# SamArgt/AudioSourceSep

Measured on AMD Instinct MI355X. Metric: Glow fwd+logdet passes/sec on 64×64×1 mel tiles (K=32,L=3), 1→8 MI355X, higher is better.
Workload: dtype f16x3

## Files before the change

audiosourcesep_amd/csrc/glowk_act_scale.h:

```cpp
#pragma once
#define GLOWK_ACT_SCALE 4.0f
```

audiosourcesep_amd/csrc/glowk_co.h:

```cpp
#pragma once
#include "glowk_kernels.h"

constexpr int CO_PX = 128;
constexpr int CO_PSTR = 132;

template <int KIN, int MOUT, int NF, int MODE>
struct RingC {
  static constexpr int MODE7 = net_dir<MODE>;
  using S = RingS<KIN, MOUT, NF, MODE7, 2>;
  static constexpr bool FUSE = (MODE & NET_FUSE) != 0;
  static constexpr bool SAVE = MODE7 == NET_FWD_SAVE, BWD = MODE7 == NET_BWD;
  static constexpr bool MERGE = S::NMT <= 3;
  static constexpr bool M0LAST = S::NMT % 3 == 2;
  static constexpr bool STORE = (MODE & NET_STORE) != 0;
  static constexpr int MODEX = net_dir<MODE> | (MODE & NET_STORE);
  static constexpr int NFH = S::NFH, NRB = S::NRB, NMT = S::NMT, KS = S::KS;
  static constexpr int UNITP = S::MAINP / 2;
  static constexpr int UNIT4 = S::MAIN4 / 2;
  static constexpr int PPW = UNITP / 4;
  static constexpr int NG = NFH / 2;
  static constexpr int K1PW = (S::K1P + 3) / 4;
  static constexpr int EPN = BWD ? 0 : S::EPN;
  static constexpr int MASKN = BWD ? 2 * 4 * NF * 64 : 0;
  static constexpr size_t LDS_BYTES = (size_t)3 * UNIT4 * 16 + (size_t)2 * S::K14 * 16 + (size_t)EPN * 4 + (size_t)MASKN * 2 +
// ... 258 lines not shown
  if constexpr (G::BWD) {
    stage4<NF / 2, 65>(reinterpret_cast<const float4*>(a.mask1 + (size_t)blockIdx.x * 4 * NF * 64), reinterpret_cast<float4*>(mkl), c.w4, c.voff);
    stage4<NF / 2, 66>(reinterpret_cast<const float4*>(a.mask2 + (size_t)blockIdx.x * 4 * NF * 64), reinterpret_cast<float4*>(mkl + 4 * NF * 64), c.w4, c.voff);
  }

  h8 xh[KS][2], xl[KS][2];
  float xmax = 0.0f;
  {
    const int hw = a.h * a.w;
#pragma unroll
    for (int hf = 0; hf < 2; ++hf) {
      const int qq = qok[hf] ? q[hf] : 0;
      const int rem = qq % hw;
      const int i = rem / a.w, j0 = rem % a.w;
      const float* base = a.vin + (long)qq * a.in_stride + a.in_off;
      if constexpr (G::BWD) {
        float v[KS][8];
        float pm = 0.0f;
#pragma unroll
        for (int s = 0; s < KS; ++s) {
          gather8<KIN, false, SGN>(base, i, j0, a.h, a.w, a.in_stride, qok[hf], 32 * s + 8 * kq, v[s]);
          pm = range8(pm, v[s]);
        }
        pm = nan_max(pm, __shfl_xor(pm, 16, 64));
        pm = nan_max(pm, __shfl_xor(pm, 32, 64));
        xmax = nan_max(xmax, pm);
        const float fac = G::STORE ? 1.0f : pixel_norm(pm, a.bnorm, hc.ub[hf]);
#pragma unroll
        for (int s = 0; s < KS; ++s) {
#pragma unroll
          for (int j = 0; j < 8; ++j) v[s][j] *= fac;
          split8(v[s], xh[s][hf], xl[s][hf]);
        }
      } else {
#pragma unroll
        for (int s = 0; s < KS; ++s) {
          float v[8];
          gather8<KIN, true, SGN>(base, i, j0, a.h, a.w, a.in_stride, qok[hf], 32 * s + 8 * kq, v);
          xmax = range8(xmax, v);
          split8(v, xh[s][hf], xl[s][hf]);
        }
      }
    }
  }
  if constexpr (G::FUSE) {
    if (tid < CO_PX) {
      const int qv = (int)blockIdx.x * CO_PX + tid;
      vstash[tid] = qv < a.Q ? *reinterpret_cast<const float4*>(a.vin + (size_t)qv * 4) : float4{0.f, 0.f, 0.f, 0.f};
    }
  }
  if constexpr (!G::BWD)
    for (int i = tid; i < S::EPN; i += 256) epl[i] = a.eph[i];
  if (((G::BWD && !G::STORE) ? !(xmax <= 3.0e38f) : !(xmax <= a.xlim)) && a.flag) *a.flag = 1;
  if (a.xmax_out) range_probe(a.xmax_out, xmax);
  asm volatile("s_waitcnt vmcnt(0)" ::: "memory");
  __syncthreads();

  f32x4 keep[G::NMT][2];
  if constexpr (SPLIT) {
    if (pass0 == 0) co_pass<KIN, MOUT, NF, MODE, 0, true>(a, hc, c, epl, plds, xh, xl, q, qok, lane, kq, keep);
    else co_pass<KIN, MOUT, NF, MODE, 1, true>(a, hc, c, epl, plds, xh, xl, q, qok, lane, kq, keep);
  } else {
    co_pass<KIN, MOUT, NF, MODE, 0, false>(a, hc, c, epl, plds, xh, xl, q, qok, lane, kq, keep);
    co_pass<KIN, MOUT, NF, MODE, 1, false>(a, hc, c, epl, plds, xh, xl, q, qok, lane, kq, keep);
  }
  if constexpr (G::FUSE) {
// ... 5 lines not shown
```

audiosourcesep_amd/csrc/glowk_kernels.h:

```cpp
#pragma once
#include "glowk_act_scale.h"

#include <hip/hip_runtime.h>
#include <utility>
#include <stdint.h>

typedef float f32x16 __attribute__((ext_vector_type(16)));

#define GLOWK_GPTR(p) ((const __attribute__((address_space(1))) void*)(p))
#define GLOWK_LPTR(p) ((__attribute__((address_space(3))) void*)(p))

__device__ __forceinline__ int mfma_row(int r, int hh) { return (r & 3) + 8 * (r >> 2) + 4 * hh; }

struct NetArgs {
  const float* vin;
  int in_stride, in_off;
  int Q, h, w;
  const float* K1p;
  const float* ep;
  const float4* R0p;
  unsigned short* mask1;
  unsigned short* mask2;
  float* P;
  size_t pstride;
// ... 430 lines not shown
  acc = __builtin_amdgcn_mfma_f32_32x32x16_f16(ahi, bhi, acc, 0, 0, 0);
  return acc;
}

template <int KIN, bool BIAS, int SGN>
__device__ __forceinline__ void gather8(const float* base, int i, int j0, int h, int w, int in_stride, bool qok, int k0, float (&v)[8]) {
  constexpr int K1 = 9 * KIN;
  constexpr int G = KIN < 8 ? KIN : 8;
  static_assert(G == 2 || G == 4 || G == 8, "channel group");
#pragma unroll
  for (int t = 0; t < 8 / G; ++t) {
    const int k = k0 + t * G;
    const int tap = k / KIN, cin = k % KIN;
    const int dy = SGN * (tap / 3 - 1), dx = SGN * (tap % 3 - 1);
    const int ii = i + dy, jj = j0 + dx;
    const bool ok = qok && k < K1 && ii >= 0 && ii < h && jj >= 0 && jj < w;
    const float* p = base + (ok ? (dy * w + dx) * in_stride + cin : 0);
    float x[G];
    if constexpr (G == 8) {
      const float4 a = *reinterpret_cast<const float4*>(p), b = *(reinterpret_cast<const float4*>(p) + 1);
      x[0] = a.x; x[1] = a.y; x[2] = a.z; x[3] = a.w; x[4] = b.x; x[5] = b.y; x[6] = b.z; x[7] = b.w;
    } else if constexpr (G == 4) {
      const float4 a = *reinterpret_cast<const float4*>(p);
      x[0] = a.x; x[1] = a.y; x[2] = a.z; x[3] = a.w;
    } else {
      const float2 a = *reinterpret_cast<const float2*>(p);
      x[0] = a.x; x[1] = a.y;
    }
#pragma unroll
    for (int e = 0; e < G; ++e) v[t * G + e] = ok ? x[e] * GLOWK_ACT_SCALE : ((BIAS && k + e == K1) ? GLOWK_ACT_SCALE : 0.0f);
  }
}

__device__ __forceinline__ void h3_barrier() {
  asm volatile("" ::: "memory");
  __builtin_amdgcn_s_barrier();
  asm volatile("" ::: "memory");
}
__device__ __forceinline__ void h3_wait_barrier() {
  __builtin_amdgcn_s_waitcnt(0x0F70);
  h3_barrier();
}

struct H3Ctx;
template <int MODE, int PASS, int NSTV = 16> __device__ __forceinline__ void h3_x_end(const H3Ctx& c);

struct H3Ctx {
  float4 *sA, *sB, *sD, *k1s0, *k1s1;
  const float4 *k1img, *img;
  const unsigned short* mkl;
  int mk2off;
  size_t wblk;
  bool wok;
  int w4;
  unsigned voff;
  float* pl;
  float ub[2];
};

template <int MODE>
__device__ __forceinline__ unsigned h3_act(const f32x16& acc, float sc, unsigned mask, h8 (&bh)[2], h8 (&bl)[2], bool do_st = false,
                                           float* st_blk = nullptr, unsigned st_lane = 0, unsigned st_row = 0, float stu = 1.0f) {
  unsigned bits = 0;
  const unsigned long long st_base = reinterpret_cast<unsigned long long>(st_blk);
#pragma unroll
  for (int s = 0; s < 2; ++s) {
// ... 304 lines not shown

  if (g) h3_barrier();
  if constexpr (SPLIT) {
    if (solo_pass == 0) h3_pass<KIN, MOUT, NF, MODE, NP, 0, 0, true>(a, c, epl, xh, xl, g, q, qok, lane, hh);
    else if (solo_pass == 1) h3_pass<KIN, MOUT, NF, MODE, NP, 0, 1, true>(a, c, epl, xh, xl, g, q, qok, lane, hh);
    else if constexpr (NP > 2) {
      if (solo_pass == 2) h3_pass<KIN, MOUT, NF, MODE, NP, 0, 2, true>(a, c, epl, xh, xl, g, q, qok, lane, hh);
      else h3_pass<KIN, MOUT, NF, MODE, NP, 0, 3, true>(a, c, epl, xh, xl, g, q, qok, lane, hh);
    }
  } else {
    h3_passes<KIN, MOUT, NF, MODE, NP, 0, 0>(a, c, epl, xh, xl, g, q, qok, lane, hh);
  }
  if (!g) h3_barrier();
}

typedef float f32x4 __attribute__((ext_vector_type(4)));

constexpr int FUSE_PSTR = 260;
constexpr int FUSE_EW = 64;

template <int KIN, int MOUT, int NF, int MODE, int NP>
struct RingS {
  static constexpr bool BWD = net_dir<MODE> == NET_BWD;
  static constexpr bool FUSE = (MODE & NET_FUSE) != 0;
  static constexpr int PXH = (MODE & NET_HALF) ? 1 : 2;
  static constexpr int NFH = NF / NP;
  static constexpr int NRB = 2 * NFH;
  static constexpr int K1 = 9 * KIN;
  static constexpr int KS = (K1 + (BWD ? 0 : 1) + 31) / 32;
  static constexpr int MAINP = NRB * 2;
  static constexpr int MAIN4 = MAINP * 64;
  static constexpr int K1P = KS * 4;
  static constexpr int K14 = K1P * 64;
  static constexpr int M3 = MOUT;
  static constexpr int NMT = (M3 + 15) / 16;
  static constexpr int TPC = MAINP / 2;
  static constexpr int NT = NFH * NMT;
  static constexpr int NCH = (NT + TPC - 1) / TPC;
  static constexpr int G0N = NMT < 6 ? NMT : 6;
  static constexpr int NGRP = (NMT + 5) / 6;
  static constexpr int GT = NFH * 6;
  static constexpr int grp_n(int gi) { return NMT - 6 * gi < 6 ? NMT - 6 * gi : 6; }
  static constexpr int EPN = (NF * 32 + 16 * NMT + 3) & ~3;
  static constexpr int MASK2B = BWD ? 2 * NF * 512 * 2 : 0;
  static constexpr size_t LDS_BYTES = (size_t)3 * MAIN4 * 16 + (size_t)2 * K14 * 16 + (size_t)EPN * 4 + MASK2B;
  static constexpr bool FITS = LDS_BYTES <= 160 * 1024 && NF % 4 == 0 && NFH >= 2 && KS <= (PXH == 1 ? (NP == 2 ? 5 : 9) : NP == 2 ? 3 : 5) && NGRP <= 3 &&
                               (NGRP == 1 || GT % TPC == 0) &&
                               (!FUSE || (MOUT == 36 && NP == 2 && PXH == 2 && LDS_BYTES + (size_t)36 * FUSE_PSTR * 4 + 4096 + 128 <= 160 * 1024));
  static constexpr int K1TOT4 = NF * K14;
  static constexpr int IMGH = NF / 2;
  static constexpr int IMG_MAIN4 = IMGH * 256;
  static constexpr int IMG_NCH = (IMGH * NMT + 2 * IMGH - 1) / (2 * IMGH);
  static constexpr int IMG_PASS4 = (NF + IMG_NCH) * IMG_MAIN4;
  static constexpr int SUBS = NP / 2;
  __device__ static const float4* main_chunk(const float4* img, int pass, int ch) {
    return img + K1TOT4 + (size_t)(pass / SUBS) * IMG_PASS4 + (size_t)ch * IMG_MAIN4 + (size_t)(pass % SUBS) * MAIN4;
  }
  __device__ static const float4* out_chunk(const float4* img, int pass, int s) {
    const int sub = pass % SUBS, t4 = s * TPC;
    const int gi = t4 / GT;
    const int t2 = IMGH * 6 * gi + sub * NFH * grp_n(gi) + (t4 - GT * gi);
    return img + K1TOT4 + (size_t)(pass / SUBS) * IMG_PASS4 + (size_t)NF * IMG_MAIN4 + (size_t)t2 * 128;
  }
  static constexpr int tile_fo(int t) { return (t - GT * (t / GT)) / grp_n(t / GT); }
  static constexpr int tile_mt(int t) { return 6 * (t / GT) + (t - GT * (t / GT)) % grp_n(t / GT); }
  static constexpr bool MERGE = PXH == 2 && NP == 2 && NGRP == 1 && NMT <= 3 &&
// ... 50 lines not shown
}
template <int MODE, bool ST>
__device__ __forceinline__ unsigned h3s_act_pair(const f32x4& r00, const f32x4& r10, const f32x4& r01, const f32x4& r11, float sc, unsigned mask16,
                                                 h8 (&bh)[2], h8 (&bl)[2], float* st_blk, unsigned st_lane, unsigned st_row) {
  float v0[8], v1[8];
  unsigned bits = h3s_act_vals<MODE>(r00, r10, sc, mask16, v0);
  bits |= h3s_act_vals<MODE>(r01, r11, sc, mask16 >> 8, v1) << 8;
  if constexpr (ST) {
    const unsigned long long st_base = reinterpret_cast<unsigned long long>(st_blk);
#pragma unroll
    for (int j = 0; j < 8; ++j) {
      const unsigned off = st_lane + (unsigned)((j >> 2) * 16 + (j & 3)) * st_row;
      const f32x2 pr = {v0[j], v1[j]};
      asm volatile("global_store_dwordx2 %0, %1, %2" GLOWK_ST_MOD ::"v"(off), "v"(pr), "s"(st_base) : "memory");
    }
  }
  split8(v0, bh[0], bl[0]);
  split8(v1, bh[1], bl[1]);
  return bits;
}

template <int KIN, int MOUT, int NF, int MODE, int NP, int KP, int PASS, bool PAIR = false>
__device__ __forceinline__ void h3s_X(const NetArgs& a, const H3Ctx& c, int fi, const h8 (&xh)[(RingS<KIN, MOUT, NF, MODE, NP>::KS)][2],
                                      const h8 (&xl)[(RingS<KIN, MOUT, NF, MODE, NP>::KS)][2], int lane, h8 (&bh)[2], h8 (&bl)[2]) {
  using G = RingS<KIN, MOUT, NF, MODE, NP>;
  unsigned mask = 0;
  if (net_dir<MODE> == NET_BWD) mask = c.mkl[c.mk2off + ((size_t)(threadIdx.x >> 6) * NF + fi) * 64 + lane];
  f32x4 h1[2][2];
#pragma unroll
  for (int i = 0; i < 4; ++i)
#pragma unroll
    for (int r = 0; r < 4; ++r) h1[i >> 1][i & 1][r] = 0.0f;
  const h8* k1 = reinterpret_cast<const h8*>(KP ? c.k1s1 : c.k1s0) + lane;
  if constexpr (G::KS <= 3) {
    h8 kf[G::K1P];
#pragma unroll
    for (int i = 0; i < G::K1P; ++i) kf[i] = k1[i * 64];
    __builtin_amdgcn_sched_barrier(0);
#pragma unroll
    for (int s = 0; s < G::KS; ++s)
#pragma unroll
      for (int rb = 0; rb < 2; ++rb)
#pragma unroll
        for (int hf = 0; hf < G::PXH; ++hf)
          h1[rb][hf] = mfma3s<net_dir<MODE> == NET_FWD2>(kf[(s * 2 + rb) * 2 + 0], kf[(s * 2 + rb) * 2 + 1], xh[s][hf], xl[s][hf], h1[rb][hf]);
  } else {
#pragma unroll
    for (int s = 0; s < G::KS; ++s)
#pragma unroll
      for (int rb = 0; rb < 2; ++rb) {
        const h8 ah = k1[((s * 2 + rb) * 2 + 0) * 64], al = k1[((s * 2 + rb) * 2 + 1) * 64];
#pragma unroll
        for (int hf = 0; hf < G::PXH; ++hf) h1[rb][hf] = mfma3s<net_dir<MODE> == NET_FWD2>(ah, al, xh[s][hf], xl[s][hf], h1[rb][hf]);
      }
  }
  unsigned bits = 0;
  if constexpr (PAIR) {
    static_assert(G::PXH == 2, "pairs: two pixel halves per wave");
    const int stq = (int)c.wblk * 32 + 2 * (lane & 15);
    if constexpr ((MODE & NET_STORE) && PASS == 0)
      bits = h3s_act_pair<net_dir<MODE>, true>(h1[0][0], h1[1][0], h1[0][1], h1[1][1], a.sc1, mask, bh, bl, uniform_fptr(a.st1 + (size_t)fi * 32 * a.Q),
                                            ((unsigned)(4 * (lane >> 4)) * (unsigned)a.Q + (unsigned)stq) * 4u, (unsigned)a.Q * 4u);
    else bits = h3s_act_pair<net_dir<MODE>, false>(h1[0][0], h1[1][0], h1[0][1], h1[1][1], a.sc1, mask, bh, bl, nullptr, 0u, 0u);
  } else {
#pragma unroll
    for (int hf = 0; hf < G::PXH; ++hf) {
      const int stq = (int)c.wblk * (16 * G::PXH) + 16 * hf + (lane & 15);
// ... 307 lines not shown
    stage4<G::K1P, 62>(c.k1img, k1slot0, c.w4, c.voff);
    stage4<G::K1P, 63>(c.k1img + G::K14, k1slot1, c.w4, c.voff);
    if (net_dir<MODE> == NET_BWD)
      stage4<NF, 65>(reinterpret_cast<const float4*>(a.mask2 + (size_t)blockIdx.x * 8 * NF * 64), reinterpret_cast<float4*>(mkl + 8 * NF * 64), c.w4, c.voff);
  }
  h8 xh[KS][2], xl[KS][2];
  float xmax = 0.0f;
  {
    const int hw = a.h * a.w;
#pragma unroll
    for (int hf = 0; hf < G::PXH; ++hf) {
      const int qq = qok[hf] ? q[hf] : 0;
      const int rem = qq % hw;
      const int i = rem / a.w, j0 = rem % a.w;
      const float* base = a.vin + (long)qq * a.in_stride + a.in_off;
      if constexpr (net_dir<MODE> == NET_BWD) {
        float v[KS][8];
        float pm = 0.0f;
#pragma unroll
        for (int s = 0; s < KS; ++s) {
          gather8<KIN, false, SGN>(base, i, j0, a.h, a.w, a.in_stride, qok[hf], 32 * s + 8 * kq, v[s]);
          pm = range8(pm, v[s]);
        }
        pm = nan_max(pm, __shfl_xor(pm, 16, 64));
        pm = nan_max(pm, __shfl_xor(pm, 32, 64));
        xmax = nan_max(xmax, pm);
        const float fac = (MODE & NET_STORE) ? 1.0f : pixel_norm(pm, a.bnorm, c.ub[hf]);
#pragma unroll
        for (int s = 0; s < KS; ++s) {
#pragma unroll
          for (int j = 0; j < 8; ++j) v[s][j] *= fac;
          split8(v[s], xh[s][hf], xl[s][hf]);
        }
      } else {
#pragma unroll
        for (int s = 0; s < KS; ++s) {
          float v[8];
          gather8<KIN, true, SGN>(base, i, j0, a.h, a.w, a.in_stride, qok[hf], 32 * s + 8 * kq, v);
          xmax = range8(xmax, v);
          split8(v, xh[s][hf], xl[s][hf]);
        }
      }
    }
  }
  if constexpr (G::FUSE) {
    if (tid < 256) {
      const int qv = (int)blockIdx.x * 256 + tid;
      vstash[tid] = qv < a.Q ? *reinterpret_cast<const float4*>(a.vin + (size_t)qv * 4) : float4{0.f, 0.f, 0.f, 0.f};
    }
  }
  if (net_dir<MODE> != NET_BWD)
    for (int i = tid; i < G::EPN; i += 512) epl[i] = a.eph[i];
  if (((net_dir<MODE> == NET_BWD && !(MODE & NET_STORE)) ? !(xmax <= 3.0e38f) : !(xmax <= a.xlim)) && a.flag) *a.flag = 1;
  if (a.xmax_out) range_probe(a.xmax_out, xmax);
  asm volatile("s_waitcnt vmcnt(0)" ::: "memory");
  __syncthreads();

  f32x4 keep[G::G0N][2];
  if (g) h3_barrier();
  if constexpr (SPLIT) {
    if (solo_pass == 0) h3s_pass<KIN, MOUT, NF, MODE, NP, 0, 0, true>(a, c, epl, xh, xl, g, q, qok, lane, kq, keep);
    else if (solo_pass == 1) h3s_pass<KIN, MOUT, NF, MODE, NP, 0, 1, true>(a, c, epl, xh, xl, g, q, qok, lane, kq, keep);
    else if constexpr (NP > 2) {
      if (solo_pass == 2) h3s_pass<KIN, MOUT, NF, MODE, NP, 0, 2, true>(a, c, epl, xh, xl, g, q, qok, lane, kq, keep);
      else h3s_pass<KIN, MOUT, NF, MODE, NP, 0, 3, true>(a, c, epl, xh, xl, g, q, qok, lane, kq, keep);
    }
// ... 11 lines not shown
```

audiosourcesep_amd/csrc/glowk_pack.h:

```cpp
#pragma once
#include "../../include/glowk.h"
#include "glowk_act_scale.h"

#include <algorithm>
#include <atomic>
#include <cmath>
#include <cstring>
#include <string>
#include <thread>
#include <vector>

#ifndef __HIP__
struct float4;
#endif

namespace {

inline uint16_t f32_to_f16(float f) {
  uint32_t x;
  std::memcpy(&x, &f, 4);
  const uint16_t sign = (uint16_t)((x >> 16) & 0x8000u);
  const uint32_t em = x & 0x7FFFFFFFu;
  if (em >= 0x7F800000u) return (uint16_t)(sign | (em > 0x7F800000u ? 0x7E00u : 0x7C00u));
  if (em >= 0x477FF000u) return (uint16_t)(sign | 0x7C00u);
// ... 290 lines not shown
              v = K3[((size_t)tap * F + f) * CO + co];
            }
            dst[L.R0p + (size_t)(NF + mt) * L.slot0 + idx] = v;
          }
  if (L.k1f0) {
    const size_t mainf = (size_t)NF * 1024, k1n = (size_t)KS1 * 64;
    for (int c2 = 0; c2 < NF + NMT; ++c2) {
      const int k1blk = (c2 < NF) ? (c2 + 1) % NF : 0;
      std::memcpy(dst + L.R0p + (size_t)c2 * L.slot0 + mainf, dst + L.K1p + (size_t)k1blk * k1n, k1n * 4);
    }
  }
  for (int i = 0; i < 6; ++i) scales3[i] = 1.0f;
  scales3[6] = scales3[7] = 0.0f;
  const double RANGE_LIM = 60000.0 / (double)GLOWK_ACT_SCALE;
  auto pow2_scale = [](const float* w, size_t n) {
    float m = 0.0f;
    for (size_t i = 0; i < n; ++i) m = std::fmax(m, std::fabs(w[i]));
    int e = 0;
    if (m > 0.0f) { std::frexp(m, &e); }
    return 14 - e;
  };
  const F16Codes QC = f16_code_bases(c, F);
  auto put = [dst, f16_map](float* row_lane, int j, int hl, float w, int S) {
    if (f16_map) {
      f16_map[(size_t)(row_lane - dst) * 2 + (size_t)hl * 512 + j] = (int)w | (hl << 30);
      return;
    }
    const float ws = std::ldexp(w, S);
    const uint16_t hi = f32_to_f16(ws);
    const uint16_t lo = f32_to_f16(ws - f16_to_f32(hi));
    uint16_t* dsth = reinterpret_cast<uint16_t*>(row_lane) + (size_t)hl * 64 * 8;
    dsth[j] = hl ? lo : hi;
  };
  if (L.slotH || L.slotS) {
    const int KS = (9 * CI + 1 + 15) / 16;
    std::vector<float> K1f((size_t)(9 * CI + 1) * F), K2f((size_t)F * F), K3f((size_t)9 * F * CO);
    std::vector<double> b2f(F), pbf((size_t)9 * CO, 0.0);
    std::vector<int> e1(F), e2(F);
    {
      const float* ep = dst + L.ep;
      std::vector<double> m1(F), m2(F);
      for (int f = 0; f < F; ++f) {
        int e;
        m1[f] = std::frexp((double)ep[F + f], &e);      e1[f] = ep[F + f] != 0.0f ? e : 0;
        m2[f] = std::frexp((double)ep[4 * F + f], &e);  e2[f] = ep[4 * F + f] != 0.0f ? e : 0;
      }
      for (int kk = 0; kk <= 9 * CI; ++kk)
        for (int f = 0; f < F; ++f)
          K1f[(size_t)kk * F + f] = std::ldexp(kk < 9 * CI ? K1[(size_t)kk * F + f] : ep[f], e1[f]);
      for (int fo = 0; fo < F; ++fo) b2f[fo] = (double)ep[3 * F + fo];
      for (int fi = 0; fi < F; ++fi)
        for (int fo = 0; fo < F; ++fo) {
          const double w = (double)K2[(size_t)fi * F + fo];
          K2f[(size_t)fi * F + fo] = (float)std::ldexp(w * m1[fi], e2[fo]);
          b2f[fo] += w * (double)ep[2 * F + fi];
        }
      for (int tap = 0; tap < 9; ++tap)
        for (int f = 0; f < F; ++f)
          for (int co = 0; co < CO; ++co) {
            const double w = (double)K3[((size_t)tap * F + f) * CO + co];
            K3f[((size_t)tap * F + f) * CO + co] = (float)(w * m2[f]);
            pbf[(size_t)tap * CO + co] += w * (double)ep[5 * F + f];
          }
    }
    {
      const float* ep = dst + L.ep;
// ... 47 lines not shown
            put(row_lane, j, 1, w, S1);
          }
    if (L.slotH)
    for (int ps = 0; ps < 2; ++ps)
      for (int ch = 0; ch < NF + NMT; ++ch) {
        float* chunk = img + (size_t)NF * k1blk + ((size_t)ps * (NF + NMT) + ch) * chunkf;
        for (int tp = 0; tp < NFH; ++tp)
          for (int s2 = 0; s2 < 2; ++s2)
            for (int l = 0; l < 64; ++l)
              for (int j = 0; j < 8; ++j) {
                const int i = l & 31, hh = l >> 5;
                const int kloc = 16 * s2 + 8 * (j >> 2) + 4 * hh + (j & 3);
                float w = 0.0f;
                int S;
                if (ch < NF) { w = K2f[(size_t)(ch * 32 + kloc) * F + (ps * NFH + tp) * 32 + i]; S = S2; }
                else {
                  const int t = (ch - NF) * NFH + tp;
                  const int fo = t < NFH * G0N ? t / G0N : (t - NFH * G0N) / G1N;
                  const int mt = t < NFH * G0N ? t % G0N : G0N + (t - NFH * G0N) % G1N;
                  const int m = mt * 32 + i, f = (ps * NFH + fo) * 32 + kloc;
                  S = S3;
                  if (m < 9 * CO) { const int tap = m / CO, co = m % CO; w = K3f[((size_t)tap * F + f) * CO + co]; }
                }
                float* row_lane = chunk + ((size_t)((tp * 2 + s2) * 2) * 64 + l) * 4;
                put(row_lane, j, 0, w, S);
                put(row_lane, j, 1, w, S);
              }
      }
    if (L.slotS) {
      const int KSS = (9 * CI + 1 + 31) / 32, NMS = (18 * CI + 15) / 16, NRB = 2 * NFH, TPC = 2 * NFH, NT = NFH * NMS;
      const int NCH = (NT + TPC - 1) / TPC;
      const size_t k1blkS = (size_t)KSS * 4 * 256;
      float* imgS = dst + L.RSp;
      for (int blk = 0; blk < NF; ++blk)
        for (int s2 = 0; s2 < KSS; ++s2)
          for (int rb = 0; rb < 2; ++rb)
            for (int l = 0; l < 64; ++l)
              for (int j = 0; j < 8; ++j) {
                const int i = l & 15, kq = l >> 4, kk = 32 * s2 + 8 * kq + j;
                const float w = kk <= 9 * CI ? K1f[(size_t)kk * F + blk * 32 + rb * 16 + i] : 0.0f;
                float* row_lane = imgS + (size_t)blk * k1blkS + ((size_t)((s2 * 2 + rb) * 2) * 64 + l) * 4;
                put(row_lane, j, 0, w, S1);
                put(row_lane, j, 1, w, S1);
              }
      for (int ps = 0; ps < 2; ++ps)
        for (int ch = 0; ch < NF + NCH; ++ch) {
          float* chunk = imgS + (size_t)NF * k1blkS + ((size_t)ps * (NF + NCH) + ch) * chunkf;
          for (int tp = 0; tp < NRB; ++tp)
            for (int l = 0; l < 64; ++l)
              for (int j = 0; j < 8; ++j) {
                const int i = l & 15, kq = l >> 4;
                const int kloc = 16 * (j >> 2) + 4 * kq + (j & 3);
                float w = 0.0f;
                int S = S2;
                if (ch < NF) w = K2f[(size_t)(ch * 32 + kloc) * F + ps * NFH * 32 + tp * 16 + i];
                else {
                  const int t = (ch - NF) * TPC + tp;
                  S = S3;
                  if (t < NT) {
                    const int gi = t / (NFH * 6), gn = NMS - 6 * gi < 6 ? NMS - 6 * gi : 6, tl = t - gi * NFH * 6;
                    const int fo = tl / gn, mt = 6 * gi + tl % gn;
                    const int m = mt * 16 + i, f = (ps * NFH + fo) * 32 + kloc;
                    if (m < 9 * CO) { const int tap = m / CO, co = m % CO; w = K3f[((size_t)tap * F + f) * CO + co]; }
                  }
                }
                float* row_lane = chunk + ((size_t)(tp * 2) * 64 + l) * 4;
// ... 179 lines not shown
```

audiosourcesep_amd/csrc/glowk_q.h:

```cpp
#pragma once
#include "glowk_kernels.h"

template <int KIN, int MOUT, int NF, int MODE>
struct RingQ {
  using S = RingS<KIN, MOUT, NF, MODE | NET_HALF, 4>;
  static constexpr int MODE7 = net_dir<MODE>;
  static constexpr bool BWD = MODE7 == NET_BWD;
  static constexpr int KS = S::KS, NFH = S::NFH, NRB = S::NRB;
  static constexpr int EPN = BWD ? 4 : S::EPN;
  static constexpr int MASKB = BWD ? NF * 512 * 2 : 0;
  static constexpr size_t FIXED = (size_t)5 * S::MAIN4 * 16 + (size_t)EPN * 4 + MASKB + 64;
  static constexpr int XB = ((size_t)4 * S::K14 * 16 + FIXED <= 160 * 1024) ? 2 : 1;
  static constexpr size_t LDS_BYTES = FIXED + (size_t)2 * XB * S::K14 * 16;
  static constexpr int NB = NF / XB;
  static constexpr int PPW = S::MAINP / 4;
  static constexpr int GS = NRB % 4 == 0 ? 4 : 2;
  static constexpr int XST = ((MODE7 == NET_FWD_SAVE) ? 1 : 0) + ((MODE & NET_STORE) ? 8 : 0);
  static constexpr bool FITS = S::FITS && LDS_BYTES <= 160 * 1024 && NF % (2 * XB) == 0 && NF % 4 == 0 && KS <= 5 && S::MAINP % 4 == 0 && NF >= 8 &&
                               (MODE7 == NET_FWD || MODE7 == NET_FWD_SAVE || MODE7 == NET_BWD) && !(MODE & NET_FUSE);
};

template <int N>
__device__ __forceinline__ void q_end() {
  __builtin_amdgcn_s_waitcnt((N & 15) | 0x0070 | ((N >> 4) << 14));
// ... 11 lines not shown
                                          const h8 (&xl)[(RingQ<KIN, MOUT, NF, MODE>::KS)][2], int g, int lane, h8 (&bfh)[NF / 2], h8 (&bfl)[NF / 2]) {
  using G = RingQ<KIN, MOUT, NF, MODE>;
  using S = typename G::S;
  constexpr int XB = G::XB, KS = G::KS, MODE7 = G::MODE7;
  if constexpr (B >= 1 && B + 1 < G::NB) {
    if (g) {
      stage4<S::K1P, 100 + 2 * B>(c.k1img + (size_t)((B + 1) * XB) * S::K14, sl.k[(B + 1) & 1][0], c.w4, c.voff);
      if constexpr (XB == 2) stage4<S::K1P, 101 + 2 * B>(c.k1img + (size_t)((B + 1) * XB + 1) * S::K14, sl.k[(B + 1) & 1][1], c.w4, c.voff);
    }
  }
  if constexpr (B == 0) {
    if (!g) {
      stage4<S::MAINP, 84>(S::main_chunk(c.img, PASS, 2), sl.r[2], c.w4, c.voff);
      stage4<S::MAINP, 85>(S::main_chunk(c.img, PASS, 3), sl.r[3], c.w4, c.voff);
    }
  }
  const h8* k1[2] = {reinterpret_cast<const h8*>(sl.k[B & 1][0]) + lane, reinterpret_cast<const h8*>(sl.k[B & 1][XB - 1]) + lane};
  unsigned mask[2] = {0u, 0u};
  if constexpr (G::BWD) {
#pragma unroll
    for (int x = 0; x < XB; ++x) mask[x] = sl.mk[((size_t)(threadIdx.x >> 6) * NF + B * XB + x) * 64 + lane];
  }
  f32x4 h1[2][2];
#pragma unroll
  for (int i = 0; i < 4; ++i)
#pragma unroll
    for (int r = 0; r < 4; ++r) h1[i >> 1][i & 1][r] = 0.0f;
  h8 A[2][2][2][2];
  auto load = [&](int buf, int s) {
#pragma unroll
    for (int x = 0; x < XB; ++x)
#pragma unroll
      for (int rb = 0; rb < 2; ++rb) {
        A[buf][x][rb][0] = k1[x][((s * 2 + rb) * 2 + 0) * 64];
        A[buf][x][rb][1] = k1[x][((s * 2 + rb) * 2 + 1) * 64];
      }
  };
  load(0, 0);
#pragma unroll
  for (int s = 0; s < KS; ++s) {
    if (s + 1 < KS) load((s + 1) & 1, s + 1);
    __builtin_amdgcn_sched_barrier(0);
#pragma unroll
    for (int t = 0; t < 3; ++t)
#pragma unroll
      for (int x = 0; x < XB; ++x)
#pragma unroll
        for (int rb = 0; rb < 2; ++rb) {
          const h8& av = A[s & 1][x][rb][t == 0 ? 1 : 0];
          const h8& bv = t == 1 ? xl[s][0] : xh[s][0];
          h1[x][rb] = __builtin_amdgcn_mfma_f32_16x16x32_f16(av, bv, h1[x][rb], 0, 0, 0);
        }
    __builtin_amdgcn_sched_barrier(0);
  }
#pragma unroll
  for (int x = 0; x < XB; ++x) {
    const int fi = B * XB + x;
    const int stq = (int)c.wblk * 16 + (lane & 15);
    h8 bh, bl;
    const unsigned bits = h3s_act<MODE7, (MODE & NET_STORE) != 0>(h1[x][0], h1[x][1], a.sc1, mask[x], bh, bl, (MODE & NET_STORE) && PASS == 0 && stq < a.Q,
                                                         (MODE & NET_STORE) ? uniform_fptr(a.st1 + (size_t)fi * 32 * a.Q) : nullptr,
                                                         ((unsigned)(4 * (lane >> 4)) * (unsigned)a.Q + (unsigned)stq) * 4u, (unsigned)a.Q * 4u);
    if (MODE7 == NET_FWD_SAVE && PASS == 0 && c.wok) a.mask1[(c.wblk * NF + fi) * 64 + lane] = (unsigned short)bits;
    bfh[fi % (NF / 2)] = bh;
    bfl[fi % (NF / 2)] = bl;
  }
  constexpr int NST = PASS == 0 ? XB * G::XST : 0;
  if (NST != 0 && !c.wok) q_end<0>();
  else q_end<NST>();
}

template <int KIN, int MOUT, int NF, int MODE, int PASS, int OFF, int... B>
__device__ __forceinline__ void q_X_all(const NetArgs& a, const H3Ctx& c, const QSlots& sl, const h8 (&xh)[(RingQ<KIN, MOUT, NF, MODE>::KS)][2],
                                        const h8 (&xl)[(RingQ<KIN, MOUT, NF, MODE>::KS)][2], int g, int lane, h8 (&bfh)[NF / 2], h8 (&bfl)[NF / 2],
                                        std::integer_sequence<int, B...>) {
  (q_X_batch<KIN, MOUT, NF, MODE, PASS, OFF + B>(a, c, sl, xh, xl, g, lane, bfh, bfl), ...);
}

template <int KIN, int MOUT, int NF, int MODE, int PASS, int P>
__device__ __forceinline__ void q_Y_pair(const H3Ctx& c, const QSlots& sl, const h8 (&bfh)[NF / 2], const h8 (&bfl)[NF / 2],
                                         f32x4 (&acc2)[(RingQ<KIN, MOUT, NF, MODE>::NRB)][2], int g, int lane) {
  using G = RingQ<KIN, MOUT, NF, MODE>;
  using S = typename G::S;
  constexpr int I = 2 * P, NRB = G::NRB, GS = G::GS, NGC = NRB / GS, NGRP = 2 * NGC;
  constexpr bool REQ_MAIN = P >= 1 && I + 3 < NF;
// ... 130 lines not shown
    stage4<S::K1P, 63>(c.k1img, k1e0, c.w4, c.voff);
    if constexpr (XB == 2) stage4<S::K1P, 66>(c.k1img + S::K14, k1e1, c.w4, c.voff);
    stage4<S::K1P, 67>(c.k1img + (size_t)XB * S::K14, k1o0, c.w4, c.voff);
    if constexpr (XB == 2) stage4<S::K1P, 68>(c.k1img + (size_t)(XB + 1) * S::K14, k1o1, c.w4, c.voff);
    if (G::BWD)
      stage4<NF, 65>(reinterpret_cast<const float4*>(a.mask2 + (size_t)blockIdx.x * 8 * NF * 64), reinterpret_cast<float4*>(mkl), c.w4, c.voff);
  }
  h8 xh[KS][2], xl[KS][2];
  float xmax = 0.0f;
  {
    const int hw = a.h * a.w;
    const int qq = qok[0] ? q[0] : 0;
    const int rem = qq % hw;
    const int i = rem / a.w, j0 = rem % a.w;
    const float* base = a.vin + (long)qq * a.in_stride + a.in_off;
    if constexpr (G::BWD) {
      float v[KS][8];
      float pm = 0.0f;
#pragma unroll
      for (int s = 0; s < KS; ++s) {
        gather8<KIN, false, SGN>(base, i, j0, a.h, a.w, a.in_stride, qok[0], 32 * s + 8 * kq, v[s]);
        pm = range8(pm, v[s]);
      }
      pm = nan_max(pm, __shfl_xor(pm, 16, 64));
      pm = nan_max(pm, __shfl_xor(pm, 32, 64));
      xmax = pm;
      const float fac = (MODE & NET_STORE) ? 1.0f : pixel_norm(pm, a.bnorm, c.ub[0]);
#pragma unroll
      for (int s = 0; s < KS; ++s) {
#pragma unroll
        for (int j = 0; j < 8; ++j) v[s][j] *= fac;
        split8(v[s], xh[s][0], xl[s][0]);
      }
    } else {
#pragma unroll
      for (int s = 0; s < KS; ++s) {
        float v[8];
        gather8<KIN, true, SGN>(base, i, j0, a.h, a.w, a.in_stride, qok[0], 32 * s + 8 * kq, v);
        xmax = range8(xmax, v);
        split8(v, xh[s][0], xl[s][0]);
      }
    }
#pragma unroll
    for (int s = 0; s < KS; ++s) { xh[s][1] = xh[s][0]; xl[s][1] = xl[s][0]; }
  }
  if (!G::BWD)
    for (int i = tid; i < G::EPN; i += 512) epl[i] = a.eph[i];
  if (((G::BWD && !(MODE & NET_STORE)) ? !(xmax <= 3.0e38f) : !(xmax <= a.xlim)) && a.flag) *a.flag = 1;
  if (a.xmax_out) range_probe(a.xmax_out, xmax);
  asm volatile("s_waitcnt vmcnt(0)" ::: "memory");
  __syncthreads();

  if (pass == 0) q_pass<KIN, MOUT, NF, MODE, 0>(a, c, sl, epl, xh, xl, g, q, qok, lane, kq);
  else if (pass == 1) q_pass<KIN, MOUT, NF, MODE, 1>(a, c, sl, epl, xh, xl, g, q, qok, lane, kq);
  else if (pass == 2) q_pass<KIN, MOUT, NF, MODE, 2>(a, c, sl, epl, xh, xl, g, q, qok, lane, kq);
  else q_pass<KIN, MOUT, NF, MODE, 3>(a, c, sl, epl, xh, xl, g, q, qok, lane, kq);
}
```

Baseline: 16100.

## Stack f16x3 split terms along K in first conv to cut MFMA count

For the forward first 3x3 convolution, the three split-precision products (whi*xhi, whi*xlo, wlo*xhi) are concatenated along the reduction axis into one longer K. A single chain of MFMAs over the stacked operand replaces three separate passes over K. This applies whenever the stacked length fits in at most twice the plain K-step count. It cuts MFMA issue when K1 is small and padding waste dominates. The cost is a more complex gather with per-element segment selection and a new host-side weight packing layout.

Measured after the change: 16310, median of 6. 1.3% higher.

```diff
diff --git a/audiosourcesep_amd/csrc/glowk_act_scale.h b/audiosourcesep_amd/csrc/glowk_act_scale.h
--- a/audiosourcesep_amd/csrc/glowk_act_scale.h
+++ b/audiosourcesep_amd/csrc/glowk_act_scale.h
@@ -1,2 +1,6 @@
 #pragma once
 #define GLOWK_ACT_SCALE 4.0f
+
+constexpr int glowk_conv1_ks(int K1) { return (K1 + 1 + 31) / 32; }
+constexpr int glowk_conv1_ks_stacked(int K1) { return (3 * K1 + 2 + 31) / 32; }
+constexpr bool glowk_conv1_stacked(int K1) { return glowk_conv1_ks_stacked(K1) <= 2 * glowk_conv1_ks(K1); }
diff --git a/audiosourcesep_amd/csrc/glowk_co.h b/audiosourcesep_amd/csrc/glowk_co.h
--- a/audiosourcesep_amd/csrc/glowk_co.h
+++ b/audiosourcesep_amd/csrc/glowk_co.h
@@ -314,6 +314,8 @@
           for (int j = 0; j < 8; ++j) v[s][j] *= fac;
           split8(v[s], xh[s][hf], xl[s][hf]);
         }
+      } else if constexpr (S::STK) {
+        xmax = gather_stacked<KIN, SGN, G::MODE7 == NET_FWD2, KS, S::KSX>(base, i, j0, a.h, a.w, a.in_stride, qok[hf], kq, xh, xl, hf, xmax);
       } else {
 #pragma unroll
         for (int s = 0; s < KS; ++s) {
diff --git a/audiosourcesep_amd/csrc/glowk_kernels.h b/audiosourcesep_amd/csrc/glowk_kernels.h
--- a/audiosourcesep_amd/csrc/glowk_kernels.h
+++ b/audiosourcesep_amd/csrc/glowk_kernels.h
@@ -486,6 +486,64 @@
   }
 }
 
+template <int KIN, int SGN, bool TWO>
+__device__ __forceinline__ float gather8_stacked(const float* base, int i, int j0, int h, int w, int in_stride, bool qok, int p0, h8& f, float xmax) {
+  constexpr int K1 = 9 * KIN;
+  constexpr int G = KIN < 8 ? KIN : 8;
+  static_assert(G == 2 || G == 4 || G == 8, "channel group");
+#pragma unroll
+  for (int t = 0; t < 8 / G; ++t) {
+    const int p = p0 + t * G;
+    const int seg = p / K1, k = p - seg * K1;
+    const int tap = k / KIN, cin = k % KIN;
+    const int dy = SGN * (tap / 3 - 1), dx = SGN * (tap % 3 - 1);
+    const int ii = i + dy, jj = j0 + dx;
+    const bool ok = qok && seg < 3 && ii >= 0 && ii < h && jj >= 0 && jj < w;
+    const float* ptr = base + (ok ? (dy * w + dx) * in_stride + cin : 0);
+    int okv = ok ? -1 : 0, cbv = p == 3 * K1 ? __float_as_int(GLOWK_ACT_SCALE) : 0;
+    asm volatile("" : "+v"(okv), "+v"(cbv));
+    float x[G];
+    if constexpr (G == 8) {
+      const float4 a = *reinterpret_cast<const float4*>(ptr), b = *(reinterpret_cast<const float4*>(ptr) + 1);
+      x[0] = a.x; x[1] = a.y; x[2] = a.z; x[3] = a.w; x[4] = b.x; x[5] = b.y; x[6] = b.z; x[7] = b.w;
+    } else if constexpr (G == 4) {
+      const float4 a = *reinterpret_cast<const float4*>(ptr);
+      x[0] = a.x; x[1] = a.y; x[2] = a.z; x[3] = a.w;
+    } else {
+      const float2 a = *reinterpret_cast<const float2*>(ptr);
+      x[0] = a.x; x[1] = a.y;
+    }
+#pragma unroll
+    for (int e = 0; e < G; e += 2) {
+      const int cbe = e == 0 ? cbv : 0;
+      const f32x2 v = {__int_as_float((__float_as_int(x[e] * GLOWK_ACT_SCALE) & okv) | cbe), __int_as_float((__float_as_int(x[e + 1] * GLOWK_ACT_SCALE) & okv) | cbe)};
+      xmax = nan_max(nan_max(xmax, __builtin_fabsf(v.x)), __builtin_fabsf(v.y));
+      const h2v hi = __builtin_convertvector(v, h2v);
+      const h2v lo = __builtin_convertvector(v - __builtin_convertvector(hi, f32x2), h2v);
+      const h2v z = {(_Float16)0.0f, (_Float16)0.0f};
+      const h2v sel = seg == 1 ? (TWO ? z : lo) : hi;
+      f[t * G + e] = sel[0]; f[t * G + e + 1] = sel[1];
+    }
+  }
+  return xmax;
+}
+template <int KIN, int SGN, bool TWO, int KS, int KSX>
+__device__ __forceinline__ float gather_stacked(const float* base, int i, int j0, int h, int w, int in_stride, bool qok, int kq, h8 (&xh)[KS][2],
+                                                h8 (&xl)[KS][2], int hf, float xmax) {
+#pragma unroll
+  for (int sx = 0; sx < 2 * KS; ++sx) {
+    h8& f = (sx & 1) ? xl[sx >> 1][hf] : xh[sx >> 1][hf];
+    if (sx < KSX) xmax = gather8_stacked<KIN, SGN, TWO>(base, i, j0, h, w, in_stride, qok, 32 * sx + 8 * kq, f, xmax);
+    else {
+#pragma unroll
+      for (int j = 0; j < 8; ++j) f[j] = (_Float16)0.0f;
+    }
+  }
+  return xmax;
+}
+template <int KS>
+__device__ __forceinline__ const h8& x_frag(const h8 (&xh)[KS][2], const h8 (&xl)[KS][2], int sx, int hf) { return (sx & 1) ? xl[sx >> 1][hf] : xh[sx >> 1][hf]; }
+
 __device__ __forceinline__ void h3_barrier() {
   asm volatile("" ::: "memory");
   __builtin_amdgcn_s_barrier();
@@ -856,6 +914,8 @@
   static constexpr int MAIN4 = MAINP * 64;
   static constexpr int K1P = KS * 4;
   static constexpr int K14 = K1P * 64;
+  static constexpr bool STK = !BWD && glowk_conv1_stacked(K1);
+  static constexpr int KSX = STK ? glowk_conv1_ks_stacked(K1) : KS;
   static constexpr int M3 = MOUT;
   static constexpr int NMT = (M3 + 15) / 16;
   static constexpr int TPC = MAINP / 2;
@@ -972,7 +1032,20 @@
 #pragma unroll
     for (int r = 0; r < 4; ++r) h1[i >> 1][i & 1][r] = 0.0f;
   const h8* k1 = reinterpret_cast<const h8*>(KP ? c.k1s1 : c.k1s0) + lane;
-  if constexpr (G::KS <= 3) {
+  if constexpr (G::STK) {
+    static_assert(G::KSX <= 6, "operand reads in flight");
+    h8 kf[G::KSX * 2];
+#pragma unroll
+    for (int i = 0; i < G::KSX * 2; ++i) kf[i] = k1[i * 64];
+    __builtin_amdgcn_sched_barrier(0);
+#pragma unroll
+    for (int s = 0; s < G::KSX; ++s)
+#pragma unroll
+      for (int rb = 0; rb < 2; ++rb)
+#pragma unroll
+        for (int hf = 0; hf < G::PXH; ++hf)
+          h1[rb][hf] = __builtin_amdgcn_mfma_f32_16x16x32_f16(kf[s * 2 + rb], x_frag(xh, xl, s, hf), h1[rb][hf], 0, 0, 0);
+  } else if constexpr (G::KS <= 3) {
     h8 kf[G::K1P];
 #pragma unroll
     for (int i = 0; i < G::K1P; ++i) kf[i] = k1[i * 64];
@@ -1346,6 +1419,8 @@
           for (int j = 0; j < 8; ++j) v[s][j] *= fac;
           split8(v[s], xh[s][hf], xl[s][hf]);
         }
+      } else if constexpr (G::STK) {
+        xmax = gather_stacked<KIN, SGN, net_dir<MODE> == NET_FWD2, KS, G::KSX>(base, i, j0, a.h, a.w, a.in_stride, qok[hf], kq, xh, xl, hf, xmax);
       } else {
 #pragma unroll
         for (int s = 0; s < KS; ++s) {
diff --git a/audiosourcesep_amd/csrc/glowk_pack.h b/audiosourcesep_amd/csrc/glowk_pack.h
--- a/audiosourcesep_amd/csrc/glowk_pack.h
+++ b/audiosourcesep_amd/csrc/glowk_pack.h
@@ -346,6 +346,15 @@
     uint16_t* dsth = reinterpret_cast<uint16_t*>(row_lane) + (size_t)hl * 64 * 8;
     dsth[j] = hl ? lo : hi;
   };
+  auto put_half = [dst, f16_map](float* lane16, int j, int hl, float w, int S) {
+    if (f16_map) {
+      f16_map[(size_t)(lane16 - dst) * 2 + j] = (int)w ? ((int)w | (hl << 30)) : 0;
+      return;
+    }
+    const float ws = std::ldexp(w, S);
+    const uint16_t hi = f32_to_f16(ws);
+    reinterpret_cast<uint16_t*>(lane16)[j] = hl ? f32_to_f16(ws - f16_to_f32(hi)) : hi;
+  };
   if (L.slotH || L.slotS) {
     const int KS = (9 * CI + 1 + 15) / 16;
     std::vector<float> K1f((size_t)(9 * CI + 1) * F), K2f((size_t)F * F), K3f((size_t)9 * F * CO);
@@ -459,6 +468,19 @@
       const int NCH = (NT + TPC - 1) / TPC;
       const size_t k1blkS = (size_t)KSS * 4 * 256;
       float* imgS = dst + L.RSp;
+      const int K1n = 9 * CI;
+      if (glowk_conv1_stacked(K1n)) {
+        for (int blk = 0; blk < NF; ++blk)
+          for (int s2 = 0; s2 < 2 * KSS; ++s2)
+            for (int rb = 0; rb < 2; ++rb)
+              for (int l = 0; l < 64; ++l)
+                for (int j = 0; j < 8; ++j) {
+                  const int i = l & 15, kq = l >> 4, p = 32 * s2 + 8 * kq + j;
+                  const int kk = p < 3 * K1n ? p % K1n : p <= 3 * K1n + 1 ? K1n : -1, hl = p < 3 * K1n ? (p / K1n == 2) : (p == 3 * K1n + 1);
+                  const float w = kk >= 0 ? K1f[(size_t)kk * F + blk * 32 + rb * 16 + i] : 0.0f;
+                  put_half(imgS + (size_t)blk * k1blkS + ((size_t)(s2 * 2 + rb) * 64 + l) * 4, j, hl, w, S1);
+                }
+      } else
       for (int blk = 0; blk < NF; ++blk)
         for (int s2 = 0; s2 < KSS; ++s2)
           for (int rb = 0; rb < 2; ++rb)
diff --git a/audiosourcesep_amd/csrc/glowk_q.h b/audiosourcesep_amd/csrc/glowk_q.h
--- a/audiosourcesep_amd/csrc/glowk_q.h
+++ b/audiosourcesep_amd/csrc/glowk_q.h
@@ -67,8 +67,13 @@
     for (int x = 0; x < XB; ++x)
 #pragma unroll
       for (int rb = 0; rb < 2; ++rb) {
-        A[buf][x][rb][0] = k1[x][((s * 2 + rb) * 2 + 0) * 64];
-        A[buf][x][rb][1] = k1[x][((s * 2 + rb) * 2 + 1) * 64];
+        if constexpr (S::STK) {
+          A[buf][x][rb][0] = k1[x][((2 * s) * 2 + rb) * 64];
+          A[buf][x][rb][1] = k1[x][((2 * s + 1) * 2 + rb) * 64];
+        } else {
+          A[buf][x][rb][0] = k1[x][((s * 2 + rb) * 2 + 0) * 64];
+          A[buf][x][rb][1] = k1[x][((s * 2 + rb) * 2 + 1) * 64];
+        }
       }
   };
   load(0, 0);
@@ -76,16 +81,26 @@
   for (int s = 0; s < KS; ++s) {
     if (s + 1 < KS) load((s + 1) & 1, s + 1);
     __builtin_amdgcn_sched_barrier(0);
-#pragma unroll
-    for (int t = 0; t < 3; ++t)
-#pragma unroll
-      for (int x = 0; x < XB; ++x)
-#pragma unroll
-        for (int rb = 0; rb < 2; ++rb) {
-          const h8& av = A[s & 1][x][rb][t == 0 ? 1 : 0];
-          const h8& bv = t == 1 ? xl[s][0] : xh[s][0];
-          h1[x][rb] = __builtin_amdgcn_mfma_f32_16x16x32_f16(av, bv, h1[x][rb], 0, 0, 0);
-        }
+    if constexpr (S::STK) {
+#pragma unroll
+      for (int t = 0; t < 2; ++t)
+#pragma unroll
+        for (int x = 0; x < XB; ++x)
+#pragma unroll
+          for (int rb = 0; rb < 2; ++rb)
+            if (2 * s + t < S::KSX) h1[x][rb] = __builtin_amdgcn_mfma_f32_16x16x32_f16(A[s & 1][x][rb][t], t ? xl[s][0] : xh[s][0], h1[x][rb], 0, 0, 0);
+    } else {
+#pragma unroll
+      for (int t = 0; t < 3; ++t)
+#pragma unroll
+        for (int x = 0; x < XB; ++x)
+#pragma unroll
+          for (int rb = 0; rb < 2; ++rb) {
+            const h8& av = A[s & 1][x][rb][t == 0 ? 1 : 0];
+            const h8& bv = t == 1 ? xl[s][0] : xh[s][0];
+            h1[x][rb] = __builtin_amdgcn_mfma_f32_16x16x32_f16(av, bv, h1[x][rb], 0, 0, 0);
+          }
+    }
     __builtin_amdgcn_sched_barrier(0);
   }
 #pragma unroll
@@ -282,6 +297,8 @@
         for (int j = 0; j < 8; ++j) v[s][j] *= fac;
         split8(v[s], xh[s][0], xl[s][0]);
       }
+    } else if constexpr (S::STK) {
+      xmax = gather_stacked<KIN, SGN, false, KS, S::KSX>(base, i, j0, a.h, a.w, a.in_stride, qok[0], kq, xh, xl, 0, xmax);
     } else {
 #pragma unroll
       for (int s = 0; s < KS; ++s) {
```
